# tzjtatata/Myriad

Measured on AMD Instinct MI355X. Metric: images/sec fine-tune step (Vicuna-7B + LoRA-style adapters, 224px), higher is better.
Workload: dtype bf16

## Files before the change

myriad_amd/csrc/attn_seq.hip:

```cpp
#include "attn_frag.h"
#include <cstdlib>

#define AS_D 128
#define AS_RS 144
#define AS_MAXF 10
#define AS_NW 8

struct AttnSeqParams {
  const bf16_t* qkv;
  bf16_t* o;
  float* lse;
  const int* pos;
  const float* cos_tab;
  const float* sin_tab;
  const int* kv_len;
  int B, H, S, ld, ldo;
  float scale;
  const bf16_t* o_in;
  const float* dout;
  const bf16_t* dout_bf;
  int nslab; long slab; int ldd;
  bf16_t* dqkv;
  long long* trace;
};
#define AS_STAMP(i) if (p.trace && blockIdx.x == 0 && blockIdx.y == 0 && (threadIdx.x == 0 || threadIdx.x == 448)) p.trace[(threadIdx.x ? 16 : 0) + (i)] = (long long)__builtin_amdgcn_s_memrealtime();

__device__ __forceinline__ void as_rope_pair(short8_t& a, short8_t& b, const float* cs, const float* sn, float sign) {
  const float4_t c0 = *reinterpret_cast<const float4_t*>(cs), c1 = *reinterpret_cast<const float4_t*>(cs + 4);
  const float4_t s0 = *reinterpret_cast<const float4_t*>(sn), s1 = *reinterpret_cast<const float4_t*>(sn + 4);
  short8_t oa, ob;
#pragma unroll
  for (int e = 0; e < 8; ++e) {
    const float c = e < 4 ? c0[e & 3] : c1[e & 3], s = e < 4 ? s0[e & 3] : s1[e & 3];
    const float x1 = bf2f((bf16_t)a[e]), x2 = bf2f((bf16_t)b[e]);
    oa[e] = (short)f2bf(x1 * c - sign * x2 * s);
    ob[e] = (short)f2bf(x2 * c + sign * x1 * s);
  }
  a = oa;
  b = ob;
}

#define AS_KIT 3
#define AS_VIT 5
struct AsStage {
  short8_t ka[AS_KIT], kb[AS_KIT], v[AS_VIT];
  int kps[AS_KIT];
};
__device__ __forceinline__ void as_stage_issue(AsStage& st, const bf16_t* kbase, const bf16_t* vbase, long ld, int S, int rows,
                                               const int* pos) {
#pragma unroll
  for (int u = 0; u < AS_KIT; ++u) {
    const int it = threadIdx.x + u * AS_NW * 64, row = it >> 3, c = (it & 7) * 8;
    st.ka[u] = (short8_t){0, 0, 0, 0, 0, 0, 0, 0};
    st.kb[u] = st.ka[u];
    st.kps[u] = 0;
    if (row < S) {
      st.kps[u] = pos[row];
      st.ka[u] = *reinterpret_cast<const short8_t*>(kbase + (long)row * ld + c);
      st.kb[u] = *reinterpret_cast<const short8_t*>(kbase + (long)row * ld + c + 64);
    }
  }
#pragma unroll
  for (int u = 0; u < AS_VIT; ++u) {
    const int it = threadIdx.x + u * AS_NW * 64, row = it >> 4, c = (it & 15) * 8;
    st.v[u] = (short8_t){0, 0, 0, 0, 0, 0, 0, 0};
    if (row < S) st.v[u] = *reinterpret_cast<const short8_t*>(vbase + (long)row * ld + c);
  }
}
__device__ __forceinline__ void as_stage_commit(AsStage& st, bf16_t* kimg, bf16_t* vimg, int S, int rows, const float* cs,
                                                const float* sn) {
#pragma unroll
  for (int u = 0; u < AS_KIT; ++u) {
    const int it = threadIdx.x + u * AS_NW * 64, row = it >> 3, c = (it & 7) * 8;
    if (row >= rows) continue;
    if (row < S) as_rope_pair(st.ka[u], st.kb[u], cs + (size_t)st.kps[u] * 64 + c, sn + (size_t)st.kps[u] * 64 + c, 1.f);
    *reinterpret_cast<short8_t*>(kimg + row * AS_RS + c) = st.ka[u];
    *reinterpret_cast<short8_t*>(kimg + row * AS_RS + c + 64) = st.kb[u];
  }
#pragma unroll
  for (int u = 0; u < AS_VIT; ++u) {
    const int it = threadIdx.x + u * AS_NW * 64, row = it >> 4, c = (it & 15) * 8;
    if (row >= rows) continue;
    *reinterpret_cast<short8_t*>(vimg + row * AS_RS + c) = st.v[u];
  }
}

template <bool ROPE>
__device__ __forceinline__ void as_row_frags(short8_t (&f)[4], const bf16_t* base, long ld, int row, int S, int lg,
                                             const int* pos, const float* cs, const float* sn) {
#pragma unroll
  for (int kk = 0; kk < 4; ++kk) {
    f[kk] = (short8_t){0, 0, 0, 0, 0, 0, 0, 0};
    if (row < S) f[kk] = *reinterpret_cast<const short8_t*>(base + (long)row * ld + kk * 32 + lg * 8);
  }
  if (ROPE && row < S) {
    const int ps = pos[row];
    as_rope_pair(f[0], f[2], cs + (size_t)ps * 64 + lg * 8, sn + (size_t)ps * 64 + lg * 8, 1.f);
    as_rope_pair(f[1], f[3], cs + (size_t)ps * 64 + 32 + lg * 8, sn + (size_t)ps * 64 + 32 + lg * 8, 1.f);
  }
}

__device__ __forceinline__ int as_own(int nf, int wave, int which) {
  const int f = which == 0 ? nf - 1 - wave : nf - 16 + wave;
  return (f >= 0 && f < nf) ? f : -1;
}

__device__ __forceinline__ int as_own_key(int nf, int wave, int which) {
  const int f = which == 0 ? wave : 15 - wave;
  return f < nf ? f : -1;
}

#define AS_NEG_INF (-__builtin_inff())

__global__ __launch_bounds__(AS_NW * 64) void attn_seq_fwd_kernel(AttnSeqParams p) {
  extern __shared__ __attribute__((aligned(16))) char smem[];
  bf16_t* Ks = reinterpret_cast<bf16_t*>(smem);
  bf16_t* Vs = Ks + AS_MAXF * 16 * AS_RS;
  const int lane = threadIdx.x & 63, wave = __builtin_amdgcn_readfirstlane(threadIdx.x >> 6);
  const int lr = lane & 15, lg = lane >> 4;
  const int b = blockIdx.x / p.H, h = blockIdx.x % p.H;
  const int S = p.S, nf = (S + 15) >> 4, W = p.H * AS_D;
  const bf16_t* qb = p.qkv + (long)b * S * p.ld + h * AS_D;
  const bf16_t* kb = qb + W;
  const bf16_t* vb = qb + 2 * W;
  const int* pos = p.pos + (long)b * S;
  int kv_valid = p.kv_len ? p.kv_len[b] : S;
  kv_valid = kv_valid < S ? kv_valid : S;

  const int rows = ((nf + 1) & ~1) * 16;
  short8_t qa[4], qn[4];
  {
    AsStage st;
    as_stage_issue(st, kb, vb, p.ld, S, rows, pos);
    const int f0 = as_own(nf, wave, 0), f1 = as_own(nf, wave, 1);
    const int r0 = f0 >= 0 ? 16 * f0 + lr : S, r1 = f1 >= 0 ? 16 * f1 + lr : S;
    int ps0 = 0, ps1 = 0;
    if (r0 < S) ps0 = pos[r0];
    if (r1 < S) ps1 = pos[r1];
    as_row_frags<false>(qa, qb, p.ld, r0, S, lg, pos, nullptr, nullptr);
    as_row_frags<false>(qn, qb, p.ld, r1, S, lg, pos, nullptr, nullptr);
    as_stage_commit(st, Ks, Vs, S, rows, p.cos_tab, p.sin_tab);
    if (r0 < S) {
      as_rope_pair(qa[0], qa[2], p.cos_tab + (size_t)ps0 * 64 + lg * 8, p.sin_tab + (size_t)ps0 * 64 + lg * 8, 1.f);
      as_rope_pair(qa[1], qa[3], p.cos_tab + (size_t)ps0 * 64 + 32 + lg * 8, p.sin_tab + (size_t)ps0 * 64 + 32 + lg * 8, 1.f);
    }
    if (r1 < S) {
      as_rope_pair(qn[0], qn[2], p.cos_tab + (size_t)ps1 * 64 + lg * 8, p.sin_tab + (size_t)ps1 * 64 + lg * 8, 1.f);
      as_rope_pair(qn[1], qn[3], p.cos_tab + (size_t)ps1 * 64 + 32 + lg * 8, p.sin_tab + (size_t)ps1 * 64 + 32 + lg * 8, 1.f);
    }
  }
  __syncthreads();

#pragma unroll 1
  for (int which = 0; which < 2; ++which) {
    const int f = as_own(nf, wave, which);
    if (f >= 0) {
      const int qi = 16 * f + lr;
      float4_t acc[8];
#pragma unroll
      for (int jd = 0; jd < 8; ++jd) acc[jd] = (float4_t){0.f, 0.f, 0.f, 0.f};
      float mrun = AS_NEG_INF, lsum = 0.f;
#pragma unroll 1
      for (int c = 0; 2 * c <= f; ++c) {
        float4_t s[2];
        float tmax = AS_NEG_INF;
#pragma unroll
        for (int u = 0; u < 2; ++u) {
          const int j = 2 * c + u;
          s[u] = (float4_t){0.f, 0.f, 0.f, 0.f};
          if (j <= f) {
#pragma unroll
            for (int kk = 0; kk < 4; ++kk)
              s[u] = __builtin_amdgcn_mfma_f32_16x16x32_bf16(lds_frag_rm<AS_RS>(Ks, j, kk, lr, lg), qa[kk], s[u], 0, 0, 0);
          }
#pragma unroll
          for (int r = 0; r < 4; ++r) {
            const int key = 16 * j + 4 * lg + r;
            const bool ok = j <= f && key < kv_valid && key <= qi && qi < S;
            s[u][r] = ok ? s[u][r] * p.scale : AS_NEG_INF;
            tmax = fmaxf(tmax, s[u][r]);
          }
        }
        tmax = fmaxf(tmax, __shfl_xor(tmax, 16, 64));
        tmax = fmaxf(tmax, __shfl_xor(tmax, 32, 64));
        const float m_new = fmaxf(mrun, tmax);
        const float alpha = (m_new == AS_NEG_INF) ? 1.f : __expf(mrun - m_new);
        float psum = 0.f;
#pragma unroll
        for (int u = 0; u < 2; ++u)
#pragma unroll
          for (int r = 0; r < 4; ++r) {
            const float e = (m_new == AS_NEG_INF) ? 0.f : __expf(s[u][r] - m_new);
            s[u][r] = e;
            psum += e;
          }
        lsum = lsum * alpha + psum;
        mrun = m_new;
        const short8_t pb = pack8(s[0], s[1]);
#pragma unroll
        for (int jd = 0; jd < 8; ++jd) {
          acc[jd] *= alpha;
          acc[jd] = __builtin_amdgcn_mfma_f32_16x16x32_bf16(lds_frag_tr<AS_RS>(Vs, jd, c, lr, lg), pb, acc[jd], 0, 0, 0);
        }
      }
      lsum += __shfl_xor(lsum, 16, 64);
      lsum += __shfl_xor(lsum, 32, 64);
      if (qi < S) {
        const float inv = lsum > 0.f ? 1.f / lsum : 0.f;
        bf16_t* ob = p.o + ((long)b * S + qi) * p.ldo + h * AS_D;
#pragma unroll
        for (int jd = 0; jd < 8; ++jd) {
          uint2 pk;
          pk.x = pack_bf2(acc[jd][0] * inv, acc[jd][1] * inv);
          pk.y = pack_bf2(acc[jd][2] * inv, acc[jd][3] * inv);
          *reinterpret_cast<uint2*>(ob + jd * 16 + lg * 4) = pk;
        }
        if (p.lse && lg == 0) p.lse[((long)b * p.H + h) * S + qi] = (lsum > 0.f) ? mrun + __logf(lsum) : AS_NEG_INF;
      }
    }
#pragma unroll
    for (int kk = 0; kk < 4; ++kk) qa[kk] = qn[kk];
  }
}

__device__ __forceinline__ void as_dout_frags(short8_t (&f)[4], const AttnSeqParams& p, long tok, int col0, bool live, int lg) {
#pragma unroll
  for (int kk = 0; kk < 4; ++kk) f[kk] = (short8_t){0, 0, 0, 0, 0, 0, 0, 0};
  if (!live) return;
  const int col = col0 + lg * 8;
  if (p.dout_bf && p.nslab <= 1) {
#pragma unroll
    for (int kk = 0; kk < 4; ++kk) f[kk] = *reinterpret_cast<const short8_t*>(p.dout_bf + tok * p.ldd + col + kk * 32);
  } else if (p.dout_bf) {
    const bf16_t* src = p.dout_bf + tok * p.ldd + col;
    float v[4][8];
    for (int k0 = 0; k0 < p.nslab; k0 += 4) {
      short8_t h[4][4];
#pragma unroll
      for (int u = 0; u < 4; ++u)
#pragma unroll
        for (int kk = 0; kk < 4; ++kk)
          if (k0 + u < p.nslab) h[u][kk] = *reinterpret_cast<const short8_t*>(src + (long)(k0 + u) * p.slab + kk * 32);
#pragma unroll
      for (int u = 0; u < 4; ++u) {
        if (k0 + u >= p.nslab) continue;
#pragma unroll
        for (int kk = 0; kk < 4; ++kk)
#pragma unroll
          for (int e = 0; e < 8; ++e) {
            const float x = bf2f((bf16_t)h[u][kk][e]);
            if (k0 + u == 0) v[kk][e] = x; else v[kk][e] += x;
          }
      }
    }
#pragma unroll
    for (int kk = 0; kk < 4; ++kk)
      f[kk] = pack8((float4_t){v[kk][0], v[kk][1], v[kk][2], v[kk][3]}, (float4_t){v[kk][4], v[kk][5], v[kk][6], v[kk][7]});
  } else {
    const float* src = p.dout + tok * p.ldd + col;
    float4_t a[4], c[4];
    for (int k0 = 0; k0 < p.nslab; k0 += 2) {
      float4_t a2[2][4], c2[2][4];
#pragma unroll
      for (int u = 0; u < 2; ++u)
#pragma unroll
        for (int kk = 0; kk < 4; ++kk)
          if (k0 + u < p.nslab) {
            a2[u][kk] = *reinterpret_cast<const float4_t*>(src + (long)(k0 + u) * p.slab + kk * 32);
            c2[u][kk] = *reinterpret_cast<const float4_t*>(src + (long)(k0 + u) * p.slab + kk * 32 + 4);
          }
#pragma unroll
      for (int u = 0; u < 2; ++u) {
        if (k0 + u >= p.nslab) continue;
#pragma unroll
        for (int kk = 0; kk < 4; ++kk) {
          if (k0 + u == 0) { a[kk] = a2[u][kk]; c[kk] = c2[u][kk]; }
          else {
            a[kk][0] += a2[u][kk][0]; a[kk][1] += a2[u][kk][1]; a[kk][2] += a2[u][kk][2]; a[kk][3] += a2[u][kk][3];
            c[kk][0] += c2[u][kk][0]; c[kk][1] += c2[u][kk][1]; c[kk][2] += c2[u][kk][2]; c[kk][3] += c2[u][kk][3];
          }
        }
      }
    }
#pragma unroll
    for (int kk = 0; kk < 4; ++kk) f[kk] = pack8(a[kk], c[kk]);
  }
}

__device__ __forceinline__ void as_unrope_store(float4_t (&acc)[8], bf16_t* dst, bool rope, const float* cs, const float* sn,
                                                int lg) {
#pragma unroll
  for (int jd = 0; jd < 4; ++jd) {
    float4_t lo = acc[jd], hi = acc[jd + 4];
    if (rope) {
      const float4_t c = *reinterpret_cast<const float4_t*>(cs + jd * 16 + lg * 4);
      const float4_t s = *reinterpret_cast<const float4_t*>(sn + jd * 16 + lg * 4);
#pragma unroll
      for (int r = 0; r < 4; ++r) {
        const float x1 = acc[jd][r], x2 = acc[jd + 4][r];
        lo[r] = x1 * c[r] + x2 * s[r];
        hi[r] = x2 * c[r] - x1 * s[r];
      }
    }
    uint2 pk;
    pk.x = pack_bf2(lo[0], lo[1]);
    pk.y = pack_bf2(lo[2], lo[3]);
    *reinterpret_cast<uint2*>(dst + jd * 16 + lg * 4) = pk;
    pk.x = pack_bf2(hi[0], hi[1]);
    pk.y = pack_bf2(hi[2], hi[3]);
    *reinterpret_cast<uint2*>(dst + 64 + jd * 16 + lg * 4) = pk;
  }
}

__global__ __launch_bounds__(AS_NW * 64) void attn_seq_bwd_kernel(AttnSeqParams p) {
  extern __shared__ __attribute__((aligned(16))) char smem[];
  bf16_t* I0 = reinterpret_cast<bf16_t*>(smem);
  bf16_t* I1 = I0 + AS_MAXF * 16 * AS_RS;
  float* lse_s = reinterpret_cast<float*>(I1 + AS_MAXF * 16 * AS_RS);
  float* dlt_s = lse_s + AS_MAXF * 16;
  const int lane = threadIdx.x & 63, wave = __builtin_amdgcn_readfirstlane(threadIdx.x >> 6);
  const int lr = lane & 15, lg = lane >> 4;
  const int b = blockIdx.x / p.H, h = blockIdx.x % p.H;
  const int S = p.S, nf = (S + 15) >> 4, W = p.H * AS_D;
  const bf16_t* qb = p.qkv + (long)b * S * p.ld + h * AS_D;
  const bf16_t* kb = qb + W;
  const bf16_t* vb = qb + 2 * W;
  bf16_t* dqb = p.dqkv + (long)b * S * p.ld + h * AS_D;
  const int* pos = p.pos + (long)b * S;
  int kv_valid = p.kv_len ? p.kv_len[b] : S;
  kv_valid = kv_valid < S ? kv_valid : S;

  const int rows = ((nf + 1) & ~1) * 16;
  AS_STAMP(0)
  short8_t qf0[4], gf0[4], qf1[4], gf1[4], of0[4], of1[4];
  int ps0 = 0, ps1 = 0;
  float dlt0 = 0.f, dlt1 = 0.f;
  AsStage st;
  as_stage_issue(st, kb, vb, p.ld, S, rows, pos);
#pragma unroll
  for (int which = 0; which < 2; ++which) {
    short8_t (&qf)[4] = which ? qf1 : qf0;
    short8_t (&of)[4] = which ? of1 : of0;
    const int f = as_own(nf, wave, which);
    const int qi = 16 * (f < 0 ? 0 : f) + lr;
    const int row = f < 0 ? S : qi;
    if (row < S) { if (which) ps1 = pos[row]; else ps0 = pos[row]; }
    as_row_frags<false>(qf, qb, p.ld, row, S, lg, pos, nullptr, nullptr);
    as_row_frags<false>(of, p.o_in + (long)b * S * p.ldo + h * AS_D, p.ldo, row, S, lg, pos, nullptr, nullptr);
  }
  as_stage_commit(st, I0, I1, S, rows, p.cos_tab, p.sin_tab);
  AS_STAMP(1)
  for (int i = threadIdx.x; i < AS_MAXF * 16; i += AS_NW * 64) lse_s[i] = i < S ? p.lse[((long)b * p.H + h) * S + i] : 1e30f;

#pragma unroll
  for (int which = 0; which < 2; ++which) {
    short8_t (&qf)[4] = which ? qf1 : qf0;
    short8_t (&gf)[4] = which ? gf1 : gf0;
    short8_t (&of)[4] = which ? of1 : of0;
#pragma unroll
    for (int kk = 0; kk < 4; ++kk) gf[kk] = (short8_t){0, 0, 0, 0, 0, 0, 0, 0};
    const int f = as_own(nf, wave, which);
    if (f < 0) continue;
    const int qi = 16 * f + lr;
    as_dout_frags(gf, p, (long)b * S + qi, h * AS_D, qi < S, lg);
    if (qi < S) {
      const int ps = which ? ps1 : ps0;
      as_rope_pair(qf[0], qf[2], p.cos_tab + (size_t)ps * 64 + lg * 8, p.sin_tab + (size_t)ps * 64 + lg * 8, 1.f);
      as_rope_pair(qf[1], qf[3], p.cos_tab + (size_t)ps * 64 + 32 + lg * 8, p.sin_tab + (size_t)ps * 64 + 32 + lg * 8, 1.f);
    }
    float dlt = 0.f;
#pragma unroll
    for (int kk = 0; kk < 4; ++kk)
#pragma unroll
      for (int e = 0; e < 8; ++e) dlt += bf2f((bf16_t)of[kk][e]) * bf2f((bf16_t)gf[kk][e]);
    dlt += __shfl_xor(dlt, 16, 64);
    dlt += __shfl_xor(dlt, 32, 64);
    if (lg == 0) dlt_s[qi] = dlt;
    if (which) dlt1 = dlt; else dlt0 = dlt;
  }
  AS_STAMP(2)
  __syncthreads();
  AS_STAMP(3)

  const bool run_a = gridDim.y == 1 || blockIdx.y == 0, run_b = gridDim.y == 1 || blockIdx.y == 1;
#pragma unroll 1
  for (int which = 0; which < 2; ++which) {
    const int f = as_own(nf, wave, which);
    if (f >= 0 && run_a) {
      const int qi = 16 * f + lr;
      const float dlt = dlt0, lse = lse_s[qi];
      float4_t acc[8];
#pragma unroll
      for (int jd = 0; jd < 8; ++jd) acc[jd] = (float4_t){0.f, 0.f, 0.f, 0.f};
#pragma unroll 1
      for (int c = 0; 2 * c <= f; ++c) {
        float4_t ds[2];
#pragma unroll
        for (int u = 0; u < 2; ++u) {
          const int j = 2 * c + u;
          ds[u] = (float4_t){0.f, 0.f, 0.f, 0.f};
          if (j > f) continue;
          float4_t sc = {0.f, 0.f, 0.f, 0.f}, dp = {0.f, 0.f, 0.f, 0.f};
#pragma unroll
          for (int kk = 0; kk < 4; ++kk) {
            sc = __builtin_amdgcn_mfma_f32_16x16x32_bf16(lds_frag_rm<AS_RS>(I0, j, kk, lr, lg), qf0[kk], sc, 0, 0, 0);
            dp = __builtin_amdgcn_mfma_f32_16x16x32_bf16(lds_frag_rm<AS_RS>(I1, j, kk, lr, lg), gf0[kk], dp, 0, 0, 0);
          }
#pragma unroll
          for (int r = 0; r < 4; ++r) {
            const int key = 16 * j + 4 * lg + r;
            const bool ok = key < kv_valid && key <= qi && qi < S;
            const float pr = ok ? __expf(sc[r] * p.scale - lse) : 0.f;
            ds[u][r] = ok ? pr * (dp[r] - dlt) * p.scale : 0.f;
          }
        }
        const short8_t db = pack8(ds[0], ds[1]);
#pragma unroll
        for (int jd = 0; jd < 8; ++jd)
          acc[jd] = __builtin_amdgcn_mfma_f32_16x16x32_bf16(lds_frag_tr<AS_RS>(I0, jd, c, lr, lg), db, acc[jd], 0, 0, 0);
      }
      if (qi < S) {
        const int ps = pos[qi];
        as_unrope_store(acc, dqb + (long)qi * p.ld, true, p.cos_tab + (size_t)ps * 64, p.sin_tab + (size_t)ps * 64, lg);
      }
    }
#pragma unroll
    for (int kk = 0; kk < 4; ++kk) {
      const short8_t tq = qf0[kk], tg = gf0[kk];
      qf0[kk] = qf1[kk]; gf0[kk] = gf1[kk];
      qf1[kk] = tq; gf1[kk] = tg;
    }
    const float td = dlt0; dlt0 = dlt1; dlt1 = td;
  }
  AS_STAMP(4)
  if (!run_b) return;
  short8_t kf0[4], vf0[4], kf1[4], vf1[4];
#pragma unroll
  for (int which = 0; which < 2; ++which) {
    short8_t (&kf)[4] = which ? kf1 : kf0;
    short8_t (&vf)[4] = which ? vf1 : vf0;
    const int f = as_own_key(nf, wave, which);
#pragma unroll
    for (int kk = 0; kk < 4; ++kk) {
      kf[kk] = (short8_t){0, 0, 0, 0, 0, 0, 0, 0};
      vf[kk] = kf[kk];
      if (f >= 0) {
        kf[kk] = lds_frag_rm<AS_RS>(I0, f, kk, lr, lg);
        vf[kk] = lds_frag_rm<AS_RS>(I1, f, kk, lr, lg);
      }
    }
  }
  __syncthreads();
#pragma unroll
  for (int which = 0; which < 2; ++which) {
    short8_t (&qf)[4] = which ? qf1 : qf0;
    short8_t (&gf)[4] = which ? gf1 : gf0;
    const int f = as_own(nf, wave, which);
    if (f < 0) continue;
#pragma unroll
    for (int kk = 0; kk < 4; ++kk) {
      *reinterpret_cast<short8_t*>(I0 + (16 * f + lr) * AS_RS + kk * 32 + lg * 8) = qf[kk];
      *reinterpret_cast<short8_t*>(I1 + (16 * f + lr) * AS_RS + kk * 32 + lg * 8) = gf[kk];
    }
  }
  __syncthreads();
  AS_STAMP(5)
#pragma unroll 1
  for (int which = 0; which < 2; ++which) {
    const int f = as_own_key(nf, wave, which);
    if (f >= 0) {
      const int ki = 16 * f + lr;
      const bool key_ok = ki < kv_valid;
      float4_t adk[8], adv[8];
#pragma unroll
      for (int jd = 0; jd < 8; ++jd) {
        adk[jd] = (float4_t){0.f, 0.f, 0.f, 0.f};
        adv[jd] = (float4_t){0.f, 0.f, 0.f, 0.f};
      }
#pragma unroll 1
      for (int c = f >> 1; 2 * c < nf; ++c) {
        float4_t pr[2], ds[2];
#pragma unroll
        for (int u = 0; u < 2; ++u) {
          const int j = 2 * c + u;
          pr[u] = (float4_t){0.f, 0.f, 0.f, 0.f};
          ds[u] = (float4_t){0.f, 0.f, 0.f, 0.f};
          if (j < f || j >= nf) continue;
          float4_t sc = {0.f, 0.f, 0.f, 0.f}, dp = {0.f, 0.f, 0.f, 0.f};
#pragma unroll
          for (int kk = 0; kk < 4; ++kk) {
            sc = __builtin_amdgcn_mfma_f32_16x16x32_bf16(lds_frag_rm<AS_RS>(I0, j, kk, lr, lg), kf0[kk], sc, 0, 0, 0);
            dp = __builtin_amdgcn_mfma_f32_16x16x32_bf16(lds_frag_rm<AS_RS>(I1, j, kk, lr, lg), vf0[kk], dp, 0, 0, 0);
          }
          const float4_t l4 = *reinterpret_cast<const float4_t*>(lse_s + 16 * j + 4 * lg);
          const float4_t d4 = *reinterpret_cast<const float4_t*>(dlt_s + 16 * j + 4 * lg);
#pragma unroll
          for (int r = 0; r < 4; ++r) {
            const int qq = 16 * j + 4 * lg + r;
            const bool ok = key_ok && qq < S && ki <= qq;
            const float e = ok ? __expf(sc[r] * p.scale - l4[r]) : 0.f;
            pr[u][r] = e;
            ds[u][r] = ok ? e * (dp[r] - d4[r]) * p.scale : 0.f;
          }
        }
        const short8_t pb = pack8(pr[0], pr[1]), db = pack8(ds[0], ds[1]);
#pragma unroll
        for (int jd = 0; jd < 8; ++jd) {
          adv[jd] = __builtin_amdgcn_mfma_f32_16x16x32_bf16(lds_frag_tr<AS_RS>(I1, jd, c, lr, lg), pb, adv[jd], 0, 0, 0);
          adk[jd] = __builtin_amdgcn_mfma_f32_16x16x32_bf16(lds_frag_tr<AS_RS>(I0, jd, c, lr, lg), db, adk[jd], 0, 0, 0);
        }
      }
      if (ki < S) {
        const int ps = pos[ki];
        as_unrope_store(adk, dqb + W + (long)ki * p.ld, true, p.cos_tab + (size_t)ps * 64, p.sin_tab + (size_t)ps * 64, lg);
        as_unrope_store(adv, dqb + 2 * W + (long)ki * p.ld, false, nullptr, nullptr, lg);
      }
    }
#pragma unroll
    for (int kk = 0; kk < 4; ++kk) { kf0[kk] = kf1[kk]; vf0[kk] = vf1[kk]; }
  }
  AS_STAMP(6)
}

static size_t as_lds_bytes(bool bwd) {
  return (size_t)2 * AS_MAXF * 16 * AS_RS * 2 + (bwd ? 2 * AS_MAXF * 16 * 4 : 0);
}

static int as_check(int B, int H, int S, int D, int ld, int ldo) {
  if (B <= 0 || H <= 0 || S <= 0) return MH_ERR_ARG;
  if (D != AS_D || S > AS_MAXF * 16) return MH_ERR_UNSUPPORTED;
  if (ld % 8 || ldo % 8 || ld < 3 * H * D || ldo < H * D) return MH_ERR_ARG;
  return MH_OK;
}

extern "C" int mh_attn_rope_fwd(const void* qkv, int ld, void* o, int ldo, float* lse, const int* pos, const float* cos_tab,
                                const float* sin_tab, const int* kv_len, int B, int H, int S, int D, float scale,
                                hipStream_t stream) {
  int rc = as_check(B, H, S, D, ld, ldo);
  if (rc) return rc;
  if (!qkv || !o || !pos || !cos_tab || !sin_tab) return MH_ERR_ARG;
  AttnSeqParams p = {};
  p.qkv = (const bf16_t*)qkv; p.o = (bf16_t*)o; p.lse = lse; p.pos = pos; p.cos_tab = cos_tab; p.sin_tab = sin_tab;
  p.kv_len = kv_len; p.B = B; p.H = H; p.S = S; p.ld = ld; p.ldo = ldo; p.scale = scale;
  static bool attr = false;
  if (!attr) {
    (void)hipFuncSetAttribute((const void*)attn_seq_fwd_kernel, hipFuncAttributeMaxDynamicSharedMemorySize, (int)as_lds_bytes(false));
    attr = true;
  }
  hipLaunchKernelGGL(attn_seq_fwd_kernel, dim3(B * H), dim3(AS_NW * 64), as_lds_bytes(false), stream, p);
  MH_CHECK_LAUNCH();
  return MH_OK;
}

int mh_launch_attn_rope_bwd(const void* qkv, int ld, const void* o, int ldo, const void* dout, int dout_is_bf16, int nslab,
                            long slab, int ldd, const float* lse, void* dqkv, const int* pos, const float* cos_tab,
                            const float* sin_tab, const int* kv_len, int B, int H, int S, int D, float scale,
                            hipStream_t stream);

extern "C" int mh_attn_rope_bwd(const void* qkv, int ld, const void* o, int ldo, const void* dout, int ldd, const float* lse,
                                void* dqkv, const int* pos, const float* cos_tab, const float* sin_tab, const int* kv_len,
                                int B, int H, int S, int D, float scale, hipStream_t stream) {
  return mh_launch_attn_rope_bwd(qkv, ld, o, ldo, dout, 1, 1, 0, ldd, lse, dqkv, pos, cos_tab, sin_tab, kv_len, B, H, S, D, scale,
                                 stream);
}

extern "C" int mh_attn_rope_supported(int S, int D) { return (D == AS_D && S > 0 && S <= AS_MAXF * 16) ? 1 : 0; }

static long long* g_as_trace = nullptr;
#ifdef MH_DEBUG_HOOKS
extern "C" void mhdbg_set_attn_seq_trace(void* ptr) { g_as_trace = (long long*)ptr; }
#endif

int mh_launch_attn_rope_bwd(const void* qkv, int ld, const void* o, int ldo, const void* dout, int dout_is_bf16, int nslab,
                            long slab, int ldd, const float* lse, void* dqkv, const int* pos, const float* cos_tab,
                            const float* sin_tab, const int* kv_len, int B, int H, int S, int D, float scale,
                            hipStream_t stream) {
  int rc = as_check(B, H, S, D, ld, ldo);
  if (rc) return rc;
  if (!qkv || !o || !dout || !lse || !dqkv || !pos || !cos_tab || !sin_tab || nslab < 1 || (ldd % 8) || ldd < H * D)
    return MH_ERR_ARG;
  AttnSeqParams p = {};
  p.qkv = (const bf16_t*)qkv; p.o_in = (const bf16_t*)o; p.lse = const_cast<float*>(lse); p.pos = pos;
  p.cos_tab = cos_tab; p.sin_tab = sin_tab; p.kv_len = kv_len; p.B = B; p.H = H; p.S = S; p.ld = ld; p.ldo = ldo;
  p.scale = scale; p.dqkv = (bf16_t*)dqkv; p.nslab = nslab; p.slab = slab; p.ldd = ldd;
  if (dout_is_bf16) p.dout_bf = (const bf16_t*)dout;
  else p.dout = (const float*)dout;
  p.trace = g_as_trace;
  static bool attr = false;
  if (!attr) {
    (void)hipFuncSetAttribute((const void*)attn_seq_bwd_kernel, hipFuncAttributeMaxDynamicSharedMemorySize, (int)as_lds_bytes(true));
    attr = true;
  }
  const int parts = (mh_opt(MH_OPT_ATTN_BWD_SPLIT) && B * H <= 128) ? 2 : 1;
  hipLaunchKernelGGL(attn_seq_bwd_kernel, dim3(B * H, parts), dim3(AS_NW * 64), as_lds_bytes(true), stream, p);
  MH_CHECK_LAUNCH();
  return MH_OK;
}
```

myriad_amd/csrc/common.h:

```cpp
#pragma once
#include <hip/hip_runtime.h>
#include <stdint.h>

#define MH_OK 0
#define MH_ERR_ARG (-1)
#define MH_ERR_LAUNCH (-2)
#define MH_ERR_UNSUPPORTED (-3)

typedef unsigned short bf16_t;
typedef __attribute__((ext_vector_type(8))) short short8_t;
typedef __attribute__((ext_vector_type(4))) short short4_t;
typedef __attribute__((ext_vector_type(4))) float float4_t;
typedef __attribute__((ext_vector_type(16))) float float16_t;

#define MH_CHECK_LAUNCH()                                   \
  do {                                                      \
    hipError_t e__ = hipGetLastError();                     \
    if (e__ != hipSuccess) return MH_ERR_LAUNCH;            \
  } while (0)

#define MH_MAX_ALT_WS 4
struct MhScratch {
  float* ws;
  size_t bytes;
  float* alt[MH_MAX_ALT_WS];
  hipStream_t alt_stream[MH_MAX_ALT_WS];
};
extern MhScratch g_default_scratch;
extern MhScratch* g_scratch;

enum MhOpt {
  MH_OPT_SLAB_BF16 = 0,
  MH_OPT_GEMM_SKINNY,
  MH_OPT_SWIGLU_FUSED,
  MH_OPT_GELU_FUSED,
  MH_OPT_ATTN_BWD_SPLIT,
  MH_OPT_GEMM_ZERO_PAD,
  MH_OPT_GEMM256_IMPL,
  MH_OPT_LORA_NORM_FUSED,
  MH_OPT_ATTN_FULL,
  MH_OPT_LORA_WGRAD_MFMA,
  MH_OPT_GEMM_SKIP_PAD,
  MH_OPT_GEMM_SPLIT_XCD,
  MH_OPT_COUNT
};
int mh_opt(int id);

extern bool g_mh_prof_on;
void mh_prof_pre(hipStream_t s, int kernel, int M, int N, int K, int splits, int flags);
void mh_prof_post(hipStream_t s);

__device__ __forceinline__ float bf2f(bf16_t h) { return __uint_as_float(((unsigned)h) << 16); }

typedef __bf16 mh_bf2_t __attribute__((ext_vector_type(2)));
typedef float mh_f2_t __attribute__((ext_vector_type(2)));
__device__ __forceinline__ bf16_t f2bf_sw(float f) {
  unsigned u = __float_as_uint(f);
  if ((u & 0x7fffffffu) > 0x7f800000u) return (bf16_t)((u >> 16) | 0x40);
  u += 0x7fffu + ((u >> 16) & 1u);
  return (bf16_t)(u >> 16);
}
__device__ __forceinline__ bf16_t f2bf(float f) {
  const __bf16 b = (__bf16)f;
  return (bf16_t)__builtin_bit_cast(unsigned short, b);
}
__device__ __forceinline__ unsigned pack_bf2(float lo, float hi) {
  const mh_f2_t v = {lo, hi};
  const mh_bf2_t b = __builtin_convertvector(v, mh_bf2_t);
  return __builtin_bit_cast(unsigned, b);
}

__device__ __forceinline__ unsigned dropout_hash(unsigned long long seed, unsigned long long idx) {
  unsigned h = (unsigned)idx * 0x9E3779B1u + ((unsigned)seed ^ ((unsigned)(idx >> 32) * 0x85EBCA77u));
  h ^= (unsigned)(seed >> 32) & 0x7FFFFFFFu;
  h ^= h >> 16;
  h *= 0x85EBCA6Bu;
  h ^= h >> 13;
  h *= 0xC2B2AE35u;
  h ^= h >> 16;
  return h;
}
__device__ __forceinline__ unsigned dropout_hash2(unsigned h) {
  h = (h ^ 0x68E31DA4u) * 0x2C1B3C6Du;
  return h ^ (h >> 15);
}
__device__ __forceinline__ float dropout_keep(unsigned long long seed, unsigned long long idx, float p, float inv_keep) {
  if (p <= 0.f) return 1.f;
  unsigned h = dropout_hash(seed, idx);
  if (seed >> 63) h = dropout_hash2(h);
  const float u = (float)(h >> 8) * (1.0f / 16777216.0f);
  return u >= p ? inv_keep : 0.f;
}
__device__ __forceinline__ void dropout_keep_pair(unsigned long long seed, unsigned long long idx, float p, float inv_keep,
                                                  float& k0, float& k1) {
  if (p <= 0.f) { k0 = k1 = 1.f; return; }
  const unsigned h = dropout_hash(seed, idx);
  k0 = (float)(h >> 8) * (1.0f / 16777216.0f) >= p ? inv_keep : 0.f;
  k1 = (float)(dropout_hash2(h) >> 8) * (1.0f / 16777216.0f) >= p ? inv_keep : 0.f;
}

__device__ __forceinline__ float4_t slab_load4(const void* base, long idx, int slab_bf16) {
  if (slab_bf16) {
    const short4_t h = *reinterpret_cast<const short4_t*>(reinterpret_cast<const bf16_t*>(base) + idx);
    return (float4_t){bf2f((bf16_t)h[0]), bf2f((bf16_t)h[1]), bf2f((bf16_t)h[2]), bf2f((bf16_t)h[3])};
  }
  return *reinterpret_cast<const float4_t*>(reinterpret_cast<const float*>(base) + idx);
}

__device__ __forceinline__ float lora_dx_value(float base, float s, float acc, float kq, float accv, float kv) {
#pragma clang fp contract(off)
  return __builtin_fmaf(s, __builtin_fmaf(acc, kq, accv * kv), base);
}
__device__ __forceinline__ void rms_bwd_sums(float x, float w, float g, float& ss, float& dot) {
#pragma clang fp contract(off)
  ss = __builtin_fmaf(x, x, ss);
  dot = __builtin_fmaf(x * w, g, dot);
}
__device__ __forceinline__ float rms_bwd_value(float r, float w, float g, float x, float cc) {
#pragma clang fp contract(off)
  return __builtin_fmaf(-x, cc, (r * w) * g);
}

__device__ __forceinline__ float wave_sum(float v) {
#pragma unroll
  for (int o = 32; o > 0; o >>= 1) v += __shfl_xor(v, o, 64);
  return v;
}
__device__ __forceinline__ float wave_max(float v) {
#pragma unroll
  for (int o = 32; o > 0; o >>= 1) v = fmaxf(v, __shfl_xor(v, o, 64));
  return v;
}

template <int NW>
__device__ __forceinline__ float block_sum(float v, float* red) {
  v = wave_sum(v);
  if (NW == 1) return v;
  const int w = threadIdx.x >> 6, l = threadIdx.x & 63;
  __syncthreads();
  if (l == 0) red[w] = v;
  __syncthreads();
  float t = 0.f;
#pragma unroll
  for (int i = 0; i < NW; ++i) t += red[i];
  return t;
}
template <int NW>
__device__ __forceinline__ float block_max(float v, float* red) {
  v = wave_max(v);
  if (NW == 1) return v;
  const int w = threadIdx.x >> 6, l = threadIdx.x & 63;
  __syncthreads();
  if (l == 0) red[w] = v;
  __syncthreads();
  float t = red[0];
#pragma unroll
  for (int i = 1; i < NW; ++i) t = fmaxf(t, red[i]);
  return t;
}

__device__ __forceinline__ float mh_erfc_abs(float ax, float gauss ) {
  const float t = __builtin_amdgcn_rcpf(1.f + 0.3275911f * ax);
  const float poly = t * (0.254829592f + t * (-0.284496736f + t * (1.421413741f + t * (-1.453152027f + t * 1.061405429f))));
  return poly * gauss;
}
__device__ __forceinline__ float mh_norm_cdf(float u , float gauss) {
  const float half = 0.5f * mh_erfc_abs(fabsf(u), gauss);
  return u < 0.f ? half : 1.f - half;
}
__device__ __forceinline__ float gelu_erf(float x) {
  const float u = x * 0.70710678118654752440f;
  return x * mh_norm_cdf(u, __expf(-u * u));
}
__device__ __forceinline__ float gelu_erf_grad(float x) {
  const float u = x * 0.70710678118654752440f;
  const float g = __expf(-u * u);
  const float cdf = mh_norm_cdf(u, g);
  const float pdf = 0.39894228040143267794f * g;
  return cdf + x * pdf;
}
```

myriad_amd/csrc/version.hip:

```cpp
#include "common.h"
#include <stdlib.h>
#include <string.h>
extern "C" const char* mh_version(void) { return "myriad_hip 0.1 (gfx950)"; }
extern "C" int mh_target_arch(void) { return 950; }

struct MhOptEntry { const char* name; const char* env; int def; int value; };
static MhOptEntry g_opts[MH_OPT_COUNT] = {
    {"slab_bf16", "MYRIAD_SLAB_BF16", 1, -1},
    {"gemm_skinny", "MYRIAD_GEMM_SKINNY", 1, -1},
    {"swiglu_fused", "MYRIAD_SWIGLU_FUSED", 1, -1},
    {"gelu_fused", "MYRIAD_GELU_FUSED", 1, -1},
    {"attn_bwd_split", "MYRIAD_ATTN_BWD_SPLIT", 1, -1},
    {"gemm_zero_pad", "MYRIAD_GEMM_ZERO_PAD", 1, -1},
    {"gemm256_impl", "MYRIAD_GEMM256_IMPL", 1, -1},
    {"lora_norm_fused", "MYRIAD_LORA_NORM_FUSED", 1, -1},
    {"attn_full", "MYRIAD_ATTN_FULL", 1, -1},
    {"lora_wgrad_mfma", "MYRIAD_LORA_WGRAD_MFMA", 1, -1},
    {"gemm_skip_pad", "MYRIAD_GEMM_SKIP_PAD", 1, -1},
    {"gemm_split_xcd", "MYRIAD_GEMM_SPLIT_XCD", 1, -1},
};

int mh_opt(int id) {
  MhOptEntry& o = g_opts[id];
  if (o.value < 0) {
    const char* e = getenv(o.env);
    o.value = e ? (e[0] == '0' ? 0 : 1) : o.def;
  }
  return o.value;
}

static int find_opt(const char* name) {
  if (!name) return -1;
  for (int i = 0; i < MH_OPT_COUNT; ++i)
    if (!strcmp(name, g_opts[i].name)) return i;
  return -1;
}
extern "C" int mh_get_option(const char* name) {
  const int i = find_opt(name);
  return i < 0 ? MH_ERR_ARG : mh_opt(i);
}
extern "C" int mh_set_option(const char* name, int value) {
  const int i = find_opt(name);
  if (i < 0 || (value != 0 && value != 1)) return MH_ERR_ARG;
  const int prev = mh_opt(i);
  g_opts[i].value = value;
  return prev;
}
```

Measured before the change: 201.5.

## Split attention K/V staging into halves and overlap second half with compute

The sequence-attention forward kernel now stages K/V into LDS in two halves. The first half is committed before compute starts, while the second half's loads and RoPE tables are held in registers and committed after the first query fragment is processed. Query fragments are reassigned so the first pass touches only the first half of keys, with a half-width transposed read at the boundary. The goal is to hide global-load latency of the second K/V half behind the first fragment's MFMA work, at the cost of more registers, an extra barrier and new ownership logic. It is gated by a new option that is on by default.

```diff
diff --git a/myriad_amd/csrc/attn_seq.hip b/myriad_amd/csrc/attn_seq.hip
--- a/myriad_amd/csrc/attn_seq.hip
+++ b/myriad_amd/csrc/attn_seq.hip
@@ -22,7 +22,9 @@
   int nslab; long slab; int ldd;
   bf16_t* dqkv;
   long long* trace;
+  int pipe;
 };
+#define AS_ORDER() __builtin_amdgcn_sched_barrier(0)
 #define AS_STAMP(i) if (p.trace && blockIdx.x == 0 && blockIdx.y == 0 && (threadIdx.x == 0 || threadIdx.x == 448)) p.trace[(threadIdx.x ? 16 : 0) + (i)] = (long long)__builtin_amdgcn_s_memrealtime();
 
 __device__ __forceinline__ void as_rope_pair(short8_t& a, short8_t& b, const float* cs, const float* sn, float sign) {
@@ -111,6 +113,122 @@
 }
 
 #define AS_NEG_INF (-__builtin_inff())
+
+struct AsTab { float4_t c0, c1, s0, s1; };
+__device__ __forceinline__ AsTab as_tab_load(const float* cs, const float* sn) {
+  AsTab t;
+  t.c0 = *reinterpret_cast<const float4_t*>(cs); t.c1 = *reinterpret_cast<const float4_t*>(cs + 4);
+  t.s0 = *reinterpret_cast<const float4_t*>(sn); t.s1 = *reinterpret_cast<const float4_t*>(sn + 4);
+  return t;
+}
+__device__ __forceinline__ void as_rope_pair(short8_t& a, short8_t& b, const AsTab& t, float sign) {
+#pragma clang fp contract(off)
+  short8_t oa, ob;
+#pragma unroll
+  for (int e = 0; e < 8; ++e) {
+    const float c = e < 4 ? t.c0[e & 3] : t.c1[e & 3], s = e < 4 ? t.s0[e & 3] : t.s1[e & 3];
+    const float x1 = bf2f((bf16_t)a[e]), x2 = bf2f((bf16_t)b[e]);
+    oa[e] = (short)f2bf(__builtin_fmaf(x1, c, -((sign * x2) * s)));
+    ob[e] = (short)f2bf(__builtin_fmaf(x2, c, (sign * x1) * s));
+  }
+  a = oa;
+  b = ob;
+}
+__device__ __forceinline__ void as_qtab_load(AsTab (&t)[2], const float* cs, const float* sn, int ps, int lg, bool live) {
+  t[0] = as_tab_load(cs + (size_t)ps * 64 + lg * 8, sn + (size_t)ps * 64 + lg * 8);
+  t[1] = as_tab_load(cs + (size_t)ps * 64 + 32 + lg * 8, sn + (size_t)ps * 64 + 32 + lg * 8);
+}
+__device__ __forceinline__ void as_qrope(short8_t (&f)[4], const AsTab (&t)[2], bool live) {
+  as_rope_pair(f[0], f[2], t[0], 1.f);
+  as_rope_pair(f[1], f[3], t[1], 1.f);
+  if (!live) f[0] = f[1] = f[2] = f[3] = (short8_t){0, 0, 0, 0, 0, 0, 0, 0};
+}
+
+#define AS_HKIT 2
+#define AS_HVIT 3
+struct AsHalf {
+  short8_t ka[AS_HKIT], kb[AS_HKIT], v[AS_HVIT];
+  int kps[AS_HKIT];
+};
+__device__ __forceinline__ void as_half_pos(AsHalf& st, const int* pos, int S, int r0, int r1) {
+#pragma unroll
+  for (int u = 0; u < AS_HKIT; ++u) {
+    const int row = r0 + ((threadIdx.x + u * AS_NW * 64) >> 3);
+    st.kps[u] = pos[row < S ? row : S - 1];
+  }
+}
+__device__ __forceinline__ void as_half_issue(AsHalf& st, const bf16_t* kbase, const bf16_t* vbase, long ld, int S, int r0, int r1) {
+#pragma unroll
+  for (int u = 0; u < AS_HKIT; ++u) {
+    const int it = threadIdx.x + u * AS_NW * 64, row = r0 + (it >> 3), c = (it & 7) * 8;
+    const long rc = row < S ? row : S - 1;
+    st.ka[u] = *reinterpret_cast<const short8_t*>(kbase + rc * ld + c);
+    st.kb[u] = *reinterpret_cast<const short8_t*>(kbase + rc * ld + c + 64);
+  }
+#pragma unroll
+  for (int u = 0; u < AS_HVIT; ++u) {
+    const int it = threadIdx.x + u * AS_NW * 64, row = r0 + (it >> 4), c = (it & 15) * 8;
+    const long rc = row < S ? row : S - 1;
+    st.v[u] = *reinterpret_cast<const short8_t*>(vbase + rc * ld + c);
+  }
+}
+__device__ __forceinline__ void as_half_tabs(AsTab (&t)[AS_HKIT], const AsHalf& st, const float* cs, const float* sn, int S, int r0,
+                                             int r1) {
+#pragma unroll
+  for (int u = 0; u < AS_HKIT; ++u) {
+    const int it = threadIdx.x + u * AS_NW * 64, row = r0 + (it >> 3), c = (it & 7) * 8;
+    t[u] = as_tab_load(cs + (size_t)st.kps[u] * 64 + c, sn + (size_t)st.kps[u] * 64 + c);
+  }
+}
+__device__ __forceinline__ void as_half_commit(AsHalf& st, const AsTab (&t)[AS_HKIT], bf16_t* kimg, bf16_t* vimg, int S, int r0,
+                                               int r1) {
+#pragma unroll
+  for (int u = 0; u < AS_HKIT; ++u) {
+    const int it = threadIdx.x + u * AS_NW * 64, row = r0 + (it >> 3), c = (it & 7) * 8;
+    if (row >= r1) continue;
+    as_rope_pair(st.ka[u], st.kb[u], t[u], 1.f);
+    if (row >= S) st.ka[u] = st.kb[u] = (short8_t){0, 0, 0, 0, 0, 0, 0, 0};
+    *reinterpret_cast<short8_t*>(kimg + row * AS_RS + c) = st.ka[u];
+    *reinterpret_cast<short8_t*>(kimg + row * AS_RS + c + 64) = st.kb[u];
+  }
+#pragma unroll
+  for (int u = 0; u < AS_HVIT; ++u) {
+    const int it = threadIdx.x + u * AS_NW * 64, row = r0 + (it >> 4), c = (it & 15) * 8;
+    if (row >= r1) continue;
+    if (row >= S) st.v[u] = (short8_t){0, 0, 0, 0, 0, 0, 0, 0};
+    *reinterpret_cast<short8_t*>(vimg + row * AS_RS + c) = st.v[u];
+  }
+}
+
+__device__ __forceinline__ void as_row_load(short8_t (&f)[4], const bf16_t* base, long ld, int row, int S, int lg) {
+#pragma unroll
+  for (int kk = 0; kk < 4; ++kk) {
+    f[kk] = *reinterpret_cast<const short8_t*>(base + (long)(row < S ? row : S - 1) * ld + kk * 32 + lg * 8);
+  }
+}
+
+__device__ __forceinline__ int as_own_pipe(int nf, int wave, int which, bool two) {
+  if (!two) {
+    const int f = which == 0 ? nf - 1 - wave : nf - 16 + wave;
+    return (f >= 0 && f < nf) ? f : -1;
+  }
+  const int h0 = (nf + 1) >> 1;
+  if (which == 0) {
+    const int i = (0xF20143FFu >> (4 * wave)) & 15;
+    return i < h0 ? h0 - 1 - i : -1;
+  }
+  const int i = wave < 4 ? wave : (wave == 7 ? 4 : 15);
+  return i < nf - h0 ? nf - 1 - i : -1;
+}
+__device__ __forceinline__ bool as_two_stage(int pipe, int nf) { return pipe && nf >= 3; }
+
+__device__ __forceinline__ short8_t as_frag_tr(const bf16_t* img, int jd, int c, int lr, int lg, bool lo_only) {
+  if (!lo_only) return lds_frag_tr<AS_RS>(img, jd, c, lr, lg);
+  const bf16_t* q = img + (32 * c + 4 * lg + (lr >> 2)) * AS_RS + 16 * jd + 4 * (lr & 3);
+  const short4_t a = __builtin_amdgcn_ds_read_tr16_b64_v4i16((lds_short4_t*)q);
+  return (short8_t){a[0], a[1], a[2], a[3], 0, 0, 0, 0};
+}
+
 
 __global__ __launch_bounds__(AS_NW * 64) void attn_seq_fwd_kernel(AttnSeqParams p) {
   extern __shared__ __attribute__((aligned(16))) char smem[];
@@ -128,32 +246,44 @@
   kv_valid = kv_valid < S ? kv_valid : S;
 
   const int rows = ((nf + 1) & ~1) * 16;
+  const bool two = as_two_stage(p.pipe, nf);
+  const int h0 = (nf + 1) >> 1, hrow = two ? 16 * h0 : (rows < 80 ? rows : 80);
   short8_t qa[4], qn[4];
+  AsHalf s1;
+  AsTab t1[AS_HKIT], tqn[2];
+  const int f0 = as_own_pipe(nf, wave, 0, two), f1 = as_own_pipe(nf, wave, 1, two);
+  const int r0 = f0 >= 0 ? 16 * f0 + lr : S, r1 = f1 >= 0 ? 16 * f1 + lr : S;
   {
-    AsStage st;
-    as_stage_issue(st, kb, vb, p.ld, S, rows, pos);
-    const int f0 = as_own(nf, wave, 0), f1 = as_own(nf, wave, 1);
-    const int r0 = f0 >= 0 ? 16 * f0 + lr : S, r1 = f1 >= 0 ? 16 * f1 + lr : S;
+    AsHalf s0;
+    AsTab t0[AS_HKIT], tqa[2];
+    as_half_pos(s0, pos, S, 0, hrow);
+    as_half_pos(s1, pos, S, hrow, rows);
     int ps0 = 0, ps1 = 0;
-    if (r0 < S) ps0 = pos[r0];
-    if (r1 < S) ps1 = pos[r1];
-    as_row_frags<false>(qa, qb, p.ld, r0, S, lg, pos, nullptr, nullptr);
-    as_row_frags<false>(qn, qb, p.ld, r1, S, lg, pos, nullptr, nullptr);
-    as_stage_commit(st, Ks, Vs, S, rows, p.cos_tab, p.sin_tab);
-    if (r0 < S) {
-      as_rope_pair(qa[0], qa[2], p.cos_tab + (size_t)ps0 * 64 + lg * 8, p.sin_tab + (size_t)ps0 * 64 + lg * 8, 1.f);
-      as_rope_pair(qa[1], qa[3], p.cos_tab + (size_t)ps0 * 64 + 32 + lg * 8, p.sin_tab + (size_t)ps0 * 64 + 32 + lg * 8, 1.f);
-    }
-    if (r1 < S) {
-      as_rope_pair(qn[0], qn[2], p.cos_tab + (size_t)ps1 * 64 + lg * 8, p.sin_tab + (size_t)ps1 * 64 + lg * 8, 1.f);
-      as_rope_pair(qn[1], qn[3], p.cos_tab + (size_t)ps1 * 64 + 32 + lg * 8, p.sin_tab + (size_t)ps1 * 64 + 32 + lg * 8, 1.f);
-    }
+    ps0 = pos[r0 < S ? r0 : S - 1];
+    ps1 = pos[r1 < S ? r1 : S - 1];
+    as_half_issue(s0, kb, vb, p.ld, S, 0, hrow);
+    as_row_load(qa, qb, p.ld, r0, S, lg);
+    AS_ORDER();
+    as_half_tabs(t0, s0, p.cos_tab, p.sin_tab, S, 0, hrow);
+    as_qtab_load(tqa, p.cos_tab, p.sin_tab, ps0, lg, r0 < S);
+    AS_ORDER();
+    as_half_issue(s1, kb, vb, p.ld, S, hrow, rows);
+    as_row_load(qn, qb, p.ld, r1, S, lg);
+    AS_ORDER();
+    as_half_commit(s0, t0, Ks, Vs, S, 0, hrow);
+    as_qrope(qa, tqa, r0 < S);
+    AS_ORDER();
+    as_half_tabs(t1, s1, p.cos_tab, p.sin_tab, S, hrow, rows);
+    as_qtab_load(tqn, p.cos_tab, p.sin_tab, ps1, lg, r1 < S);
+  }
+  if (!two) {
+    as_half_commit(s1, t1, Ks, Vs, S, hrow, rows);
+    as_qrope(qn, tqn, r1 < S);
   }
   __syncthreads();
 
-#pragma unroll 1
-  for (int which = 0; which < 2; ++which) {
-    const int f = as_own(nf, wave, which);
+  auto run_fragment = [&](const int which) __attribute__((always_inline)) {
+    const int f = as_own_pipe(nf, wave, which, two);
     if (f >= 0) {
       const int qi = 16 * f + lr;
       float4_t acc[8];
@@ -162,6 +292,7 @@
       float mrun = AS_NEG_INF, lsum = 0.f;
 #pragma unroll 1
       for (int c = 0; 2 * c <= f; ++c) {
+        const bool lo_only = two && !which && 2 * c + 1 >= h0;
         float4_t s[2];
         float tmax = AS_NEG_INF;
 #pragma unroll
@@ -200,7 +331,7 @@
 #pragma unroll
         for (int jd = 0; jd < 8; ++jd) {
           acc[jd] *= alpha;
-          acc[jd] = __builtin_amdgcn_mfma_f32_16x16x32_bf16(lds_frag_tr<AS_RS>(Vs, jd, c, lr, lg), pb, acc[jd], 0, 0, 0);
+          acc[jd] = __builtin_amdgcn_mfma_f32_16x16x32_bf16(as_frag_tr(Vs, jd, c, lr, lg, lo_only), pb, acc[jd], 0, 0, 0);
         }
       }
       lsum += __shfl_xor(lsum, 16, 64);
@@ -218,9 +349,16 @@
         if (p.lse && lg == 0) p.lse[((long)b * p.H + h) * S + qi] = (lsum > 0.f) ? mrun + __logf(lsum) : AS_NEG_INF;
       }
     }
-#pragma unroll
-    for (int kk = 0; kk < 4; ++kk) qa[kk] = qn[kk];
-  }
+  };
+  run_fragment(0);
+#pragma unroll
+  for (int kk = 0; kk < 4; ++kk) qa[kk] = qn[kk];
+  if (two) {
+    as_half_commit(s1, t1, Ks, Vs, S, hrow, rows);
+    as_qrope(qa, tqn, r1 < S);
+    __syncthreads();
+  }
+  run_fragment(1);
 }
 
 __device__ __forceinline__ void as_dout_frags(short8_t (&f)[4], const AttnSeqParams& p, long tok, int col0, bool live, int lg) {
@@ -542,6 +680,7 @@
   AttnSeqParams p = {};
   p.qkv = (const bf16_t*)qkv; p.o = (bf16_t*)o; p.lse = lse; p.pos = pos; p.cos_tab = cos_tab; p.sin_tab = sin_tab;
   p.kv_len = kv_len; p.B = B; p.H = H; p.S = S; p.ld = ld; p.ldo = ldo; p.scale = scale;
+  p.pipe = mh_opt(MH_OPT_ATTN_SEQ_PIPE);
   static bool attr = false;
   if (!attr) {
     (void)hipFuncSetAttribute((const void*)attn_seq_fwd_kernel, hipFuncAttributeMaxDynamicSharedMemorySize, (int)as_lds_bytes(false));
diff --git a/myriad_amd/csrc/common.h b/myriad_amd/csrc/common.h
--- a/myriad_amd/csrc/common.h
+++ b/myriad_amd/csrc/common.h
@@ -42,6 +42,7 @@
   MH_OPT_LORA_WGRAD_MFMA,
   MH_OPT_GEMM_SKIP_PAD,
   MH_OPT_GEMM_SPLIT_XCD,
+  MH_OPT_ATTN_SEQ_PIPE,
   MH_OPT_COUNT
 };
 int mh_opt(int id);
diff --git a/myriad_amd/csrc/version.hip b/myriad_amd/csrc/version.hip
--- a/myriad_amd/csrc/version.hip
+++ b/myriad_amd/csrc/version.hip
@@ -18,6 +18,7 @@
     {"lora_wgrad_mfma", "MYRIAD_LORA_WGRAD_MFMA", 1, -1},
     {"gemm_skip_pad", "MYRIAD_GEMM_SKIP_PAD", 1, -1},
     {"gemm_split_xcd", "MYRIAD_GEMM_SPLIT_XCD", 1, -1},
+    {"attn_seq_pipe", "MYRIAD_ATTN_SEQ_PIPE", 1, -1},
 };
 
 int mh_opt(int id) {
```

New measurement: 201.9 (median of 4 runs). Within noise of the previous version (+0.2%).
